# control-toolbox/CTDirect.jl

Measured on AMD Instinct MI355X. Metric: NLP callback evals/s (constraints+sparse Jac), N-step Goddard, 1/2/4/8 GPU, higher is better.
Workload: dtype f64; 1 GPU; cfg2_weak: goddard / gauss_legendre_2, 10000 time steps per GPU (global grid 10000 steps, time-step sharded); fused cons!+jac_coord! on HBM-resident x; BASELINE.json configs[1] per GPU; nvar_per_gpu=110004, ncon_per_gpu=90004, nnzj_per_gpu=1110028

## Files before the change

### ctdirect.jl_amd/csrc/ctd_engine.hip

```cpp
#include <hip/hip_runtime.h>
#include <hip/hiprtc.h>
#include <dlfcn.h>

#include <cstdio>
#include <functional>
#include <map>
#include <mutex>
#include <cstdlib>
#include <cstring>
#include <memory>
#include <new>
#include <string>
#include <vector>

#include "../../include/ctdirect_hip.h"
#include "ctd_host.hpp"
#include "ctd_kernels.hpp"
#include "ctd_hess_kernels.hpp"
#include "ctd_hess_step.hpp"
#include "ctd_iter_kernels.hpp"
#include "ctd_prod_kernels.hpp"
#include "ctd_hprod_kernels.hpp"
#include "ctd_kkt_kernels.hpp"
#include "ctd_diag_kernels.hpp"
// ... 322 lines not shown
template <class Enqueue>
static int32_t host_call(ctd_handle* h, std::initializer_list<Staged<const double>> in, Enqueue&& enqueue,
                         std::initializer_list<Staged<double>> out) {
    for (const auto& a : in) if (a.host) HIP_TRY(h, a.buf.ensure(a.n));
    for (const auto& a : out) if (a.host) HIP_TRY(h, a.buf.ensure(a.n));
    for (const auto& a : in) if (a.host) HIP_TRY(h, hipMemcpyAsync(a.buf.p, a.host, sizeof(double) * a.n, hipMemcpyHostToDevice, h->stream));
    if (const int32_t st = enqueue()) return st;
    for (const auto& a : out) if (a.host) HIP_TRY(h, hipMemcpyAsync(a.host, a.buf.p, sizeof(double) * a.n, hipMemcpyDeviceToHost, h->stream));
    HIP_TRY(h, hipStreamSynchronize(h->stream));
    return CTD_OK;
}

template <class K>
static int32_t enqueue_prod_units(ctd_handle* h, const char* fn, typename K::Params& a, int dirs, int jc, DevBuf<>& partial,
                                  const JitModule& jm, int f0, const double* x_dev, bool shard) {
    ProdParams& pp = K::prod(a);
    pp.nch = (int32_t)((dirs + jc - 1) / jc);
    const int64_t blocks = ((pp.unit_end - pp.unit_begin) * (int64_t)pp.nch + 255) / 256;
    if (blocks > 0x7fffffff) return fail(h, CTD_EINVAL, std::string(fn) + ": grid too large");
    pp.nblocks = (int32_t)blocks;
    const int32_t st = partial.grow(h, blocks * kMaxNV, fn);
    if (st) return st;
    pp.partial = partial.p;
    hipError_t e = hipErrorInvalidValue;
    if (h->rt) {
        void* args[] = {&a, &x_dev};
        e = jit_launch(jm.f[f0], (int)blocks, 256, 0, h->stream, args);
        if (e == hipSuccess) e = jit_launch(jm.f[f0 + 1], 1, 64, 0, h->stream, args);
    }
    for_problem(h->model.problem, [&](auto tag) {
        using P = typename decltype(tag)::type;
        if constexpr (K::kShardForm)
            e = shard ? launch_prod_units<P, K, true>(a, x_dev, h->stream) : launch_prod_units<P, K, false>(a, x_dev, h->stream);
        else e = launch_prod_units<P, K, false>(a, x_dev, h->stream);
    });
    if (e != hipSuccess) return fail(h, CTD_EHIP, std::string(fn) + ": kernel launch: " + hipGetErrorString(e));
    return CTD_OK;
}

extern "C" {

const char* ctd_strerror(int32_t st) {
    switch (st) {
        case CTD_OK: return "ok";
        case CTD_EINVAL: return "invalid argument";
        case CTD_EGRID: return "given time grid is not strictly increasing";
        case CTD_ESCHEME: return "unknown discretization method";
        case CTD_EPATTERN: return "sparsity pattern not available";
        case CTD_EPROBLEM: return "problem not in the compiled registry";
        case CTD_ENODEVICE: return "no HIP device bound to this handle (there is no CPU fallback)";
        case CTD_EHIP: return "HIP runtime error";
        case CTD_ENOMEM: return "out of memory";
        default: return "unknown status";
    }
}

const char* ctd_last_error(const ctd_handle* h) { return h ? h->err.c_str() : g_create_err.c_str(); }

int32_t ctd_create(const ctd_desc* desc, ctd_handle** out) {
    if (!desc || !out) return fail(nullptr, CTD_EINVAL, "ctd_create: null argument");
    *out = nullptr;
    struct Del { void operator()(ctd_handle* p) const { if (p) destroy_handle(p); } };
    std::unique_ptr<ctd_handle, Del> h(new (std::nothrow) ctd_handle());
    if (!h) return fail(nullptr, CTD_ENOMEM, "ctd_create: out of memory");
    HostDesc hd{desc->problem, desc->scheme, desc->pattern_mode, desc->grid_size, desc->time_grid, desc->time_grid_len,
                desc->control_steps > 1 ? desc->control_steps : 1, desc->value_order};
    if (desc->reserved0 != 0) return fail(nullptr, CTD_EINVAL, "ctd_create: ctd_desc.reserved0 must be 0 (zero-initialise the descriptor: memset / ctd_desc d = {0})");
    std::string err;
    int st;
    try {
        st = build_model(hd, h->model, err);
    } catch (const std::bad_alloc&) {
        return fail(nullptr, CTD_ENOMEM, "ctd_create: out of memory while building the model");
    }
    if (st) return fail(nullptr, st, err);
    const Model& mo = h->model;
    if (!runtime_ocp(mo.problem)) {
        const char* bad = nullptr;
        for_problem(mo.problem, [&](auto tag) {
            using P = typename decltype(tag)::type;
            for_scheme<true>(mo.L, [&](auto t) { bad = static_layout_mismatch<P, t.sc, t.s>(mo.L); });
        });
        if (bad) return fail(nullptr, CTD_EINVAL, std::string("ctd_create: the static layout of the kernel instantiation differs from the model's layout in field '") + bad + "'");
    }
    if (mo.L.cs > 3 && desc->device >= 0 && !runtime_ocp(mo.problem))
        return fail(nullptr, CTD_EINVAL, "ctd_create: control_steps > 3 needs an OCP registered at run time (ctd_register_ocp); the compiled registry holds the midpoint kernels for 1, 2 and 3 controls per step");
    h->step_begin = desc->step_begin;
    h->step_end = desc->step_end;
    if (h->step_begin == 0 && h->step_end == 0) h->step_end = mo.L.N;
    if (h->step_begin < 0 || h->step_end > mo.L.N || h->step_begin >= h->step_end)
        return fail(nullptr, CTD_EINVAL, "ctd_create: shard [step_begin, step_end) is not inside [0, N)");
    h->tile = env_int("CTD_TILE", 0);
    h->lean_ok = env_int("CTD_LEAN", 1) ? 1 : 0;
    if (h->tile <= 0) h->tile = default_tile(mo, h->step_end - h->step_begin);
    int maxb = 256;
    for_problem(mo.problem, [&](auto tag) { maxb = decltype(tag)::type::MAXB; });
    h->rt = runtime_ocp(mo.problem);
    if (h->rt) maxb = h->rt->maxb;
    h->block = env_int("CTD_BLOCK", 0);
    if (h->block <= 0) {
        h->block = 256;
        const int64_t ntl = (h->step_end - h->step_begin + h->tile - 1) / h->tile;
        if (ntl <= 512 && mo.nch_dyn <= 1 && mo.Lseg > 0 && 320 / mo.Lseg > 256 / mo.Lseg && mo.Lseg * (320 / mo.Lseg) * 10 >= 320 * 9) h->block = 320;
    }
    if (h->block < 64 || (h->block % 64)) h->block = 256;
    if (h->block > maxb) h->block = maxb;
    mo.fill_kparams(h->kp, h->step_begin, h->step_end, h->tile);
    h->lds_bytes = (size_t)lds_doubles(h->kp) * sizeof(double);
    const int debug_stop = env_int("CTD_DEBUG_STOP", 0);
    const size_t lds_cap = h->rt ? 64 * 1024 : 80 * 1024;
    while (h->lds_bytes > lds_cap && h->tile > 1) {
        h->tile = (h->tile + 1) / 2;
        mo.fill_kparams(h->kp, h->step_begin, h->step_end, h->tile);
        h->lds_bytes = (size_t)lds_doubles(h->kp) * sizeof(double);
    }
    const bool long_mid = mo.L.sc == SC_MIDPOINT && mo.L.cs == 1;
    if (desc->device >= 0 && !h->rt && env_int("CTD_TILE", 0) <= 0 && mo.nch_dyn <= 1 && (mo.L.sc == SC_IRK || long_mid) && h->tile >= 16) {
        DeviceGuard dgq(desc->device);
        if (dgq.err == hipSuccess) {
            auto resident = [&](int tile, size_t& lds) {
                KParams kq;
                mo.fill_kparams(kq, h->step_begin, h->step_end, tile);
                lds = (size_t)lds_doubles(kq) * sizeof(double);
                int r = 0;
                for_problem(mo.problem, [&](auto tag) { r = occupancy_cons_jac<typename decltype(tag)::type>(kq, h->block, lds); });
                (void)hipGetLastError();
                return r;
            };
            size_t l0 = 0;
            const int r0 = resident(h->tile, l0);
            const int64_t ns = h->step_end - h->step_begin, cap = 256 * (int64_t)r0;
            if (r0 > 0 && (ns + h->tile - 1) / h->tile >= env_int("CTD_LONG_GRID_ROUNDS", 8) * cap && maxb >= 512 && env_int("CTD_BLOCK", 0) <= 0 &&
                env_int("CTD_LONG_GRID", 1)) {
                int tbest = h->tile;
                for (int tt = h->tile + 1; tt <= 256; ++tt) {
                    KParams kq;
                    mo.fill_kparams(kq, h->step_begin, h->step_end, tt);
                    if ((size_t)lds_doubles(kq) * sizeof(double) > (long_mid ? 74u : 64u) * 1024) break;
                    tbest = tt;
                }
                if (tbest > h->tile) {
                    h->tile = tbest;
                    h->block = 512;
                    mo.fill_kparams(h->kp, h->step_begin, h->step_end, h->tile);
                    h->lds_bytes = (size_t)lds_doubles(h->kp) * sizeof(double);
                }
            } else if (mo.L.sc == SC_IRK && r0 > 0 && (ns + h->tile - 1) / h->tile > cap) {
                int tmax = 48;
                for (; tmax > h->tile; --tmax) { size_t l = 0; if (resident(tmax, l) >= r0 && l <= lds_cap) break; }
                const int64_t rounds = (ns + (int64_t)tmax * cap - 1) / ((int64_t)tmax * cap);
                const int64_t tb = (ns + rounds * cap - 1) / (rounds * cap);
                if (tb > h->tile && tb <= tmax) {
                    h->tile = (int)tb;
                    mo.fill_kparams(h->kp, h->step_begin, h->step_end, h->tile);
                    h->lds_bytes = (size_t)lds_doubles(h->kp) * sizeof(double);
                }
            }
        }
    }
    h->grid = h->kp.ntiles + h->kp.has_edge;
    h->kp.debug_stop = debug_stop;
    h->out_mb = 8.0 * ((double)(h->step_end - h->step_begin) * (mo.L.cb + mo.Lseg + (double)mo.L.nv * mo.vr)) / 1.0e6;
    h->kp.wt_store = h->out_mb <= kWtMB ? 1 : 0;
    h->device = desc->device;
    if (h->device >= 0) {
        int ndev = 0;
        if (hipGetDeviceCount(&ndev) != hipSuccess || h->device >= ndev)
            return fail(nullptr, CTD_ENODEVICE, "ctd_create: HIP device not available");
        ctd_handle* hp = h.get();
        if (h->lds_bytes > 160 * 1024) return fail(nullptr, CTD_EINVAL, "ctd_create: tile does not fit the 160 KiB LDS");
        DeviceGuard dg_(hp->device); HIP_TRY(nullptr, dg_.err);
        if (desc->stream_mode == CTD_STREAM_GIVEN) { hp->stream = (hipStream_t)desc->stream; hp->own_stream = false; }
        else { HIP_TRY(nullptr, hipStreamCreateWithFlags(&hp->stream, hipStreamNonBlocking)); hp->own_stream = true; }
        HIP_TRY(nullptr, upload(hp->d_tau, mo.tau));
        HIP_TRY(nullptr, upload(hp->d_tmpl, mo.tmpl));
        HIP_TRY(nullptr, upload(hp->d_vtmpl, mo.vtmpl));
        HIP_TRY(nullptr, upload(hp->d_edge_idx, mo.edge_idx));
        HIP_TRY(nullptr, upload(hp->d_edge_code, mo.edge_code));
        hp->kp.tau = hp->d_tau.p;
        hp->kp.tmpl = hp->d_tmpl.p;
        hp->kp.vtmpl = hp->d_vtmpl.p;
        {
            const int S = mo.L.s, r_dyn = S * mo.nch_dyn, r_path = mo.nch_path;
            int lgT = 0;
            while ((1 << lgT) < hp->tile) ++lgT;
            const int leadbase = (((r_dyn + r_path) << lgT) + 63) & ~63;
            const int early_lanes = mo.n_early + mo.c_early + mo.L.nv * mo.vr_early;
            if (env_int("CTD_EARLY", 0) && mo.n_early > 0 && !hp->rt && mo.fused && hp->tile <= 32 && leadbase + 64 <= hp->block && early_lanes <= 64 &&
                mo.n_late > 0 && mo.n_late <= hp->block) {
                HIP_TRY(nullptr, upload(hp->d_pos, mo.pos_order));
                hp->kp.pos = hp->d_pos.p;
                hp->kp.n_late = mo.n_late; hp->kp.n_early = mo.n_early; hp->kp.c_early = mo.c_early; hp->kp.vr_early = mo.vr_early;
                hp->kp.div_late = make_fastdiv((uint32_t)mo.n_late);
            }
        }
        hp->kp.edge_idx = hp->d_edge_idx.p;
        hp->kp.edge_code = hp->d_edge_code.p;
        hp->obj_blocks = 256;
        HIP_TRY(nullptr, hp->d_partial.ensure(hp->obj_blocks));
        HIP_TRY(nullptr, hp->d_obj.ensure(1));
        HIP_TRY(nullptr, hipEventCreate(&hp->ev0));
        HIP_TRY(nullptr, hipEventCreate(&hp->ev1));
        if (hp->rt) {
            if (hp->lds_bytes > 64 * 1024) return fail(nullptr, CTD_EINVAL, "ctd_create: one step of this run-time OCP does not fit 64 KiB of LDS");
            const int32_t jst = jit_load(hp, JIT_FIRST);
            if (jst) return jst;
        }
        {
            const bool direct = mo.fused && mo.L.sc != SC_TRAPEZE;
            const int mt = env_int("CTD_MULTI_TILE", 0);
            if (!direct && mt > 0 && kMultiTileLoop && !hp->rt) {
                int per_cu = mt > 1 ? mt : 0, cus = 256;
                if (hipDeviceGetAttribute(&cus, hipDeviceAttributeMultiprocessorCount, hp->device) != hipSuccess) cus = 256;
                if (per_cu == 0) {
                    if (hp->rt) {
                        if (hipModuleOccupancyMaxActiveBlocksPerMultiprocessor(&per_cu, hp->jit[JIT_FIRST].f[0], hp->block, hp->lds_bytes) != hipSuccess) per_cu = 0;
                    } else {
                        for_problem(mo.problem, [&](auto tag) {
                            using P = typename decltype(tag)::type;
                            per_cu = occupancy_cons_jac<P>(hp->kp, hp->block, hp->lds_bytes);
                        });
                    }
                }
                const int64_t cap = (int64_t)per_cu * cus - hp->kp.has_edge;
                if (cap > 0 && hp->kp.ntiles > cap) {
                    hp->kp.wg_stride = (int)cap;
                    hp->grid = hp->kp.wg_stride + hp->kp.has_edge;
                }
            }
        }
    }
    *out = h.release();
    return CTD_OK;
}

int32_t ctd_register_ocp(const ctd_ocp_def* def, int32_t* problem_id) {
    if (!def || !problem_id) return fail(nullptr, CTD_EINVAL, "ctd_register_ocp: null argument");
    std::string err;
    int id = -1;
    const int st = register_runtime_ocp(def, &id, err);
    if (st) return fail(nullptr, st, "ctd_register_ocp: " + err);
    *problem_id = id;
    return CTD_OK;
}

int32_t ctd_ocp_source(int32_t problem_id, char* buf, int64_t cap) {
// ... 1587 lines not shown
```

### ctdirect.jl_amd/csrc/ctd_kernel_body.hpp

```cpp
#pragma once
#include "ctd_layout.hpp"


namespace ctd {

#if defined(CTD_SUBSTAMPS) && defined(__HIP_DEVICE_COMPILE__)
#ifndef CTD_SUB_WAVE0
#define CTD_SUB_WAVE0 0
#endif
#define CTD_SUB(kp, id)                                                                                              \
    do {                                                                                                             \
        __builtin_amdgcn_sched_barrier(0);                                                                           \
        __builtin_amdgcn_s_waitcnt(0);                                                                               \
        if ((kp).stamps && (threadIdx.x & 63) == 0 && threadIdx.x >= 64 * CTD_SUB_WAVE0 && threadIdx.x < 64 * CTD_SUB_WAVE0 + 128) \
            (kp).stamps[(size_t)gridDim.x * 12 + ((size_t)blockIdx.x * 2 + (threadIdx.x >> 6) - CTD_SUB_WAVE0) * 8 + (id)] = clock64(); \
        __builtin_amdgcn_sched_barrier(0);                                                                           \
    } while (0)
#else
#define CTD_SUB(kp, id) do { } while (0)
#endif
#if defined(CTD_SUBSTAMPS_EMIT) && defined(__HIP_DEVICE_COMPILE__)
#define CTD_SUBE(kp, id)                                                                                             \
    do {                                                                                                             \
        __builtin_amdgcn_sched_barrier(0);                                                                           \
// ... 1521 lines not shown
#pragma unroll
                        for (int u = 0; u < 4; ++u) {
                            const int s = s0 + u * par;
                            if (s < nreg) emit_store(&out[s * Ls + k], a[u] * b[u] + beta, kp.wt_store);
                        }
                    }
                }
            } else {
                uint32_t code = (hp && tid < Ls) ? pre_->b : (tid < Ls ? cx.codes[tid] : 0u);
                int q = 0;
                for (int k = tid; k < Ls; k += nthr, ++q) {
                    uint32_t nxt = 0u;
                    bool have = false;
                    if constexpr (NB > 1) {
                        if (hp && q < NB - 1) {
                            have = true;
#pragma unroll
                            for (int e = 0; e < NB - 1; ++e)
                                if (e == q) nxt = pre_->more[e];
                        }
                    }
                    if (!have) nxt = k + nthr < Ls ? cx.codes[k + nthr] : 0u;
                    const int bt = code_beta(code);
                    const double beta = bt == 0 ? 0.0 : (bt == 1 ? 1.0 : -1.0);
                    const double* pc = cx.rec + (sl0 - code_crec(code)) * stride + R.oC + code_ci(code);
                    const double* pd = cx.rec + (sl0 - code_drec(code)) * stride + code_di(code);
                    const int last = nreg - 1;
                    for (int s0 = 0; s0 < nreg; s0 += 4) {
                        double a[4], b[4];
#pragma unroll
                        for (int u = 0; u < 4; ++u) {
                            const int s = s0 + u < last ? s0 + u : last;
                            a[u] = pc[s * stride];
                            b[u] = pd[s * stride];
                        }
#pragma unroll
                        for (int u = 0; u < 4; ++u)
                            if (s0 + u < nreg) emit_store(&out[(s0 + u) * Ls + k], a[u] * b[u] + beta, kp.wt_store);
                    }
                    code = nxt;
                }
            }
        }
    }
    CTD_SUBE(kp, 2);
    if (kp.vr > 0) {
        const int vr = kp.vr;
        const int par = (int)fast_div((uint32_t)nthr, kp.div_vr);
#pragma unroll
        for (int kk = 0; kk < P::NV; ++kk) {
            double* out = out_vals<B>(kp, bl) + kp.vcol_base[kk] + cx.a * (int64_t)vr;
            const uint32_t* codes = cx.vcodes + kk * vr;
            if (par >= 1) {
                if (tid < par * vr) {
                    const int g = (int)fast_div((uint32_t)tid, kp.div_vr), k = tid - g * vr;
                    const uint32_t code = hp ? pre_->v[kk] : codes[k];
                    const double* pc = cx.rec + (slot0 + g) * stride + R.oC + code_ci(code);
                    const double* pd = cx.rec + (slot0 + g) * stride + code_di(code);
                    const int adv = par * stride;
                    if (LEAN || k >= kp.vr_early)
                        for (int s = g; s < nsteps; s += par, pc += adv, pd += adv) emit_store(&out[s * vr + k], (*pc) * (*pd), kp.wt_store);
                }
            } else {
                for (int k = tid; k < vr; k += nthr) {
                    const uint32_t code = codes[k];
                    const double* pc = cx.rec + slot0 * stride + R.oC + code_ci(code);
                    const double* pd = cx.rec + slot0 * stride + code_di(code);
                    for (int s = 0; s < nsteps; ++s, pc += stride, pd += stride) emit_store(&out[s * vr + k], (*pc) * (*pd), kp.wt_store);
                }
            }
        }
    }
    CTD_SUBE(kp, 3);
}
template <class P, int SC, int S, int NB = 1, bool B = false, bool LEAN = false>
CTD_HD void phase_emit(const KParams& kp, const BlockCtx& cx, int tid, int nthr, const EmitPreT<NB>* pre = nullptr,
                       const BatchLd bl = BatchLd{}) {
    if (pre != nullptr) phase_emit_impl<P, SC, S, NB, B, LEAN>(kp, cx, tid, nthr, *pre, pre->have != 0, bl);
    else phase_emit_impl<P, SC, S, NB, B, LEAN>(kp, cx, tid, nthr, EmitPreT<NB>{}, false, bl);
}

}

#if !defined(__HIPCC_RTC__)
#include "ctd_problems.hpp"
#include "ctd_sym_registry.hpp"
#endif
```

### ctdirect.jl_amd/csrc/ctd_kernels.hpp

```cpp
#pragma once
#if !defined(__HIPCC_RTC__)
#include <hip/hip_runtime.h>
#include <hip/hip_ext.h>
#endif

#include "ctd_kernel_body.hpp"
#if !defined(__HIPCC_RTC__)
#include "ctd_problems.hpp"
#endif

namespace ctd {

#ifndef CTD_MULTI_TILE_LOOP
#define CTD_MULTI_TILE_LOOP 0
#endif
constexpr bool kMultiTileLoop = CTD_MULTI_TILE_LOOP != 0;

template <bool DBG>
__device__ __forceinline__ void ctd_stamp(const KParams& kp, int slot) {
    if constexpr (DBG) {
        if (kp.stamps && threadIdx.x == 0) {
            unsigned long long* p = kp.stamps + ((size_t)blockIdx.x * 6 + slot) * 2;
            p[0] = wall_clock64();
            p[1] = clock64();
// ... 41 lines not shown

template <class P, int SC, int S, bool DBG, bool B = false, bool LEAN = false>
__device__ __forceinline__ void cons_jac_body(const KParams& kp, const double* __restrict__ xu, int block, double* ctd_lds,
                                              const BatchLd bl = BatchLd{}) {
    if constexpr (B) xu += batch_member() * bl.ldx;
    ctd_pin_kernargs<SC == SC_IRK ? S : 0, LEAN>(kp, xu);
    ctd_stamp<DBG>(kp, 0);
    if (DBG && kp.debug_stop == 1) return;
    const int tid = (int)threadIdx.x, nthr = (int)blockDim.x;
    if constexpr (DirectTile<P, SC>::value) {
        const BlockCtx cx = make_direct_ctx<LEAN>(kp, block, ctd_lds, xu, LV<P, SC, S, LEAN>::blk(kp), LEAN ? P::NV : -1);
        const EmitPre pre = emit_prefetch<P, 1, LEAN>(kp, cx, tid, nthr);
        ctd_stamp<DBG>(kp, 1);
        phase_eval<P, SC, S, RegEval<P, SC, S>::value, 1, B, LEAN>(kp, cx, tid, nthr, &pre, bl);
        ctd_pin_emit_kernargs<LEAN>(kp);
        __syncthreads();
        ctd_stamp<DBG>(kp, 2);
        ctd_stamp<DBG>(kp, 3);
        if (DBG && kp.debug_stop >= 2 && kp.debug_stop <= 4) return;
        phase_emit<P, SC, S, 1, B, LEAN>(kp, cx, tid, nthr, &pre, bl);
        ctd_stamp<DBG>(kp, 4);
        if (DBG && kp.stamps) {
            __builtin_amdgcn_s_waitcnt(0);
            __syncthreads();
            ctd_stamp<DBG>(kp, 5);
        }
        return;
    }
    BlockCtx cx = make_ctx<LEAN>(kp, block, ctd_lds);
    constexpr int NB = EmitN<P, SC, S>::value;
    EmitPreT<NB> pre = {};
    const bool use_pre = !cx.is_edge && !codes_staged(kp);
    if (use_pre) pre = emit_prefetch<P, NB, LEAN>(kp, cx, tid, nthr);
    phase_load<P, SC, S, true, LEAN>(kp, cx, xu, tid, nthr);
    const int nblk = kp.ntiles + kp.has_edge;
    for (;;) {
        __syncthreads();
        ctd_stamp<DBG>(kp, 1);
        if (DBG && kp.debug_stop == 2) return;
        phase_eval<P, SC, S, false, 1, B, LEAN>(kp, cx, tid, nthr, nullptr, bl);
        ctd_pin_emit_kernargs<LEAN>(kp);
        __syncthreads();
        ctd_stamp<DBG>(kp, 2);
        if (DBG && kp.debug_stop == 3) return;
        if (!Dirs<P>::FUSED && !fin_folded<P, SC, S>(cx)) {
            phase_fin<P, SC, S>(kp, cx, tid, nthr);
            __syncthreads();
        }
        if (SC == SC_TRAPEZE) {
            phase_fin2<P, SC, S>(kp, cx, tid, nthr);
            __syncthreads();
        }
        ctd_stamp<DBG>(kp, 3);
        if (DBG && kp.debug_stop == 4) return;
        block += kp.wg_stride;
        const bool more = kMultiTileLoop && kp.wg_stride > 0 && !cx.is_edge && block < nblk;
        BlockCtx nx = cx;
        TileIn tin{0.0, 0.0, 0.0};
        if (more) {
            nx = make_ctx<LEAN>(kp, block, ctd_lds);
            tin = load_issue<P>(kp, nx, xu, tid, nthr);
        }
        phase_emit_impl<P, SC, S, NB, B, LEAN>(kp, cx, tid, nthr, pre, use_pre, bl);
        ctd_stamp<DBG>(kp, 4);
        if (!more) break;
        load_commit<P, SC, S>(kp, nx, xu, tin, tid, nthr);
        cx = nx;
    }
    if (DBG && kp.stamps) {
        __builtin_amdgcn_s_waitcnt(0);
        __syncthreads();
        ctd_stamp<DBG>(kp, 5);
    }
}

template <class P, int SC, int S> struct MinWaves {
    static constexpr int value = (P::NX <= 12 && !(SC == SC_MIDPOINT && S > 1)) ? 4 : 1;
};

template <class P, int SC, int S, bool DBG, bool LEAN = false>
__global__ void __launch_bounds__(P::MAXB, (MinWaves<P, SC, S>::value)) cons_jac_kernel(const KParams kp, const double* __restrict__ xu) {
    extern __shared__ double ctd_lds[];
    cons_jac_body<P, SC, S, DBG, false, LEAN>(kp, xu, (int)blockIdx.x, ctd_lds);
}
template <class P, int SC, int S>
__global__ void __launch_bounds__(P::MAXB, (MinWaves<P, SC, S>::value)) cons_jac_batch_kernel(const KParams kp, const double* __restrict__ xu,
                                                                                          const BatchLd bl) {
    extern __shared__ double ctd_lds[];
    cons_jac_body<P, SC, S, false, true>(kp, xu, (int)blockIdx.x, ctd_lds, bl);
}

struct ObjParams {
    Layout L;
    const double* tau;
    int64_t unit_begin, unit_end;
    int32_t add_mayer;
    double* partial;
    double* out;
    int32_t nblocks;
    const XHalo* halo;
    XNear near;
    int64_t ldx;
};

template <class P> __device__ double obj_time(const ObjParams& op, const double* v, int64_t i) {
    const double t0 = (P::IT0 >= 0) ? v[P::IT0 >= 0 ? P::IT0 : 0] : op.L.t0;
    const double tf = (P::ITF >= 0) ? v[P::ITF >= 0 ? P::ITF : 0] : op.L.tf;
    const double tau = op.tau ? op.tau[i] : (double)i / (double)op.L.N;
    return t0 + tau * (tf - t0);
}

template <class P, int SC>
__device__ double lagrange_unit(const ObjParams& op, const double* __restrict__ xu, const double* v, int64_t i) {
    constexpr int n = P::NX, m = P::NU;
    const Layout& L = op.L;
    const double* base = xu + i * (int64_t)L.blk;
    const int64_t gn = (i + 1) * (int64_t)L.blk;
    const double* nxt = ((op.halo && i + 1 >= op.unit_end) ? xnear(op.near, xu, gn) : xu) + gn;
    double x[n > 0 ? n : 1], u[m > 0 ? m : 1];
    if (SC == SC_TRAPEZE) {
        double w;
        if (i == 0) w = (obj_time<P>(op, v, 1) - obj_time<P>(op, v, 0)) / 2.0;
        else if (i == L.N) w = (obj_time<P>(op, v, L.N) - obj_time<P>(op, v, L.N - 1)) / 2.0;
        else w = (obj_time<P>(op, v, i + 1) - obj_time<P>(op, v, i - 1)) / 2.0;
        for (int c = 0; c < n; ++c) x[c] = base[c];
        for (int c = 0; c < m; ++c) u[c] = base[n + c];
        return w * P::template lagrange<double>(obj_time<P>(op, v, i), x, u, v);
    }
    const double ti = obj_time<P>(op, v, i), tip1 = obj_time<P>(op, v, i + 1);
    const double h = tip1 - ti;
    if (SC == SC_MIDPOINT) {
        if (L.cs > 1) {
            const double hi = h / (double)L.cs;
            for (int c = 0; c < n; ++c) x[c] = 0.5 * (base[c] + nxt[c]);
            double val = 0.0;
            for (int j = 1; j <= L.cs; ++j) {
                for (int c = 0; c < m; ++c) u[c] = base[n + (j - 1) * m + c];
                const double term = hi * P::template lagrange<double>(ti + ((double)j - 0.5) * hi, x, u, v);
                val = (j == 1) ? term : val + term;
            }
            return val;
        }
        for (int c = 0; c < m; ++c) u[c] = base[n + c];
        if (L.euler == 0) {
            for (int c = 0; c < n; ++c) x[c] = 0.5 * (base[c] + nxt[c]);
            return h * P::template lagrange<double>(0.5 * (ti + tip1), x, u, v);
        }
        for (int c = 0; c < n; ++c) x[c] = (L.euler == 1) ? base[c] : nxt[c];
        return h * P::template lagrange<double>(L.euler == 1 ? ti : tip1, x, u, v);
    }
    const double* K = base + n + L.cu;
    double local = 0.0;
    for (int j = 0; j < L.s; ++j) {
        for (int c = 0; c < n; ++c) {
            double xc = base[c];
            for (int l = 0; l < L.s; ++l) xc = xc + h * L.a[3 * j + l] * K[l * n + c];
            x[c] = xc;
        }
        const double* U = base + n + (L.stagewise ? j * m : 0);
        for (int c = 0; c < m; ++c) u[c] = U[c];
        const double term = L.b[j] * P::template lagrange<double>(ti + L.c[j] * h, x, u, v);
        local = (j == 0) ? term : local + term;
    }
    return h * local;
}

// ... 315 lines not shown
    const int lane = threadIdx.x & 63, wave = threadIdx.x >> 6;
    for (int k = 0; k < nv; ++k) {
        double a = gv[k];
        for (int off = 32; off > 0; off >>= 1) a += __shfl_down(a, off, 64);
        if (lane == 0) wsum[wave][k] = a;
    }
    __syncthreads();
    if (threadIdx.x == 0)
        for (int k = 0; k < nv; ++k) {
            double sacc = 0.0;
            for (int w = 0; w < (int)(blockDim.x >> 6); ++w) sacc += wsum[w][k];
            gp.partial[((size_t)mb * gp.nblocks + block) * kMaxNV + k] = sacc;
        }
}
template <class P, int SC, int S>
__global__ void __launch_bounds__(256) __attribute__((amdgpu_waves_per_eu(2))) grad_units_kernel(const GradParams gp, const double* __restrict__ xu) {
    __shared__ double wsum[4][kMaxNV];
    const int64_t mb = batch_member();
    grad_units_body<P, SC, S>(gp, xu + mb * gp.ldx, (int)blockIdx.x, wsum, mb);
}

template <class P>
__device__ __forceinline__ void grad_finish_body(const GradParams& gp, const double* __restrict__ xu, int64_t mb = 0) {
    if (threadIdx.x >= 64) return;
    constexpr int n = P::NX, nv = P::NV;
    const Layout& L = gp.L;
    const double* part = gp.partial + (size_t)mb * gp.nblocks * kMaxNV;
    double* const g = gp.g + mb * gp.ldg;
    double gvs[nv > 0 ? nv : 1];
    for (int k = 0; k < nv; ++k) {
        double sacc = 0.0;
        for (int b = threadIdx.x; b < gp.nblocks; b += 64) sacc += part[(size_t)b * kMaxNV + k];
        for (int off = 32; off > 0; off >>= 1) sacc += __shfl_down(sacc, off, 64);
        gvs[k] = sacc;
    }
    if (threadIdx.x != 0) return;
    if (P::HAS_MAYER && (gp.owns_first || gp.owns_last)) {
        double x0[n > 0 ? n : 1], xf[n > 0 ? n : 1], v[nv > 0 ? nv : 1], g0x[n > 0 ? n : 1], gfx[n > 0 ? n : 1], gmv[nv > 0 ? nv : 1];
        const double* b0 = grad_block(gp, xu, 0);
        const double* bf = grad_block(gp, xu, L.N);
        for (int c = 0; c < n; ++c) { x0[c] = b0[c]; xf[c] = bf[c]; g0x[c] = 0.0; gfx[c] = 0.0; }
        for (int k = 0; k < nv; ++k) { v[k] = xu[L.v_off + k]; gmv[k] = 0.0; }
        mayer_partials<P, 0>(x0, xf, v, g0x, gfx, gmv);
        for (int c = 0; c < n; ++c) {
            if (gp.owns_first) g[c] += g0x[c];
            if (gp.owns_last) g[L.N * (int64_t)L.blk + c] += gfx[c];
        }
        if (gp.owns_last) for (int k = 0; k < nv; ++k) gvs[k] += gmv[k];
    }
    for (int k = 0; k < nv; ++k) g[L.v_off + k] = gvs[k];
}
template <class P>
__global__ void grad_finish_kernel(const GradParams gp, const double* __restrict__ xu) {
    if (blockIdx.x != 0) return;
    const int64_t mb = batch_member();
    grad_finish_body<P>(gp, xu + mb * gp.ldx, mb);
}

#if !defined(__HIPCC_RTC__)
template <class P>
hipError_t launch_grad(const GradParams& gp, const double* xu, int grid, hipStream_t st, int batch) {
    const dim3 g(grid > 0 ? grid : 1, batch);
    if (grid > 0)
        for_scheme<false>(gp.L, [&](auto t) { grad_units_kernel<P, t.sc, t.s><<<g, 256, 0, st>>>(gp, xu); });
    grad_finish_kernel<P><<<dim3(1, batch), 64, 0, st>>>(gp, xu);
    return hipGetLastError();
}

#endif

#if !defined(__HIPCC_RTC__)
template <class P, int SC, int S, bool DBG, bool LEAN>
hipError_t launch_variant_dbg(const KParams& kp, const double* xu, int grid, int block, size_t lds_bytes, hipStream_t st,
                              hipEvent_t e0, hipEvent_t e1) {
    if (lds_bytes > 64 * 1024) {
        hipError_t e = hipFuncSetAttribute((const void*)cons_jac_kernel<P, SC, S, DBG, LEAN>, hipFuncAttributeMaxDynamicSharedMemorySize,
                                           (int)lds_bytes);
        if (e != hipSuccess) return e;
    }
    if (e0 || e1) hipExtLaunchKernelGGL((cons_jac_kernel<P, SC, S, DBG, LEAN>), dim3(grid), dim3(block), lds_bytes, st, e0, e1, 0, kp, xu);
    else cons_jac_kernel<P, SC, S, DBG, LEAN><<<grid, block, lds_bytes, st>>>(kp, xu);
    return hipGetLastError();
}
template <class P, int SC, int S>
hipError_t launch_variant(const KParams& kp, const double* xu, int grid, int block, size_t lds_bytes, hipStream_t st,
                          hipEvent_t e0, hipEvent_t e1, int lean_ok) {
    const bool dbg = kp.stamps || kp.debug_stop;
    constexpr bool kHasLean = DirectTile<P, SC>::value || SC == SC_IRK;
    if constexpr (kHasLean) {
        if (lean_ok && kp.halo == nullptr && kp.n_early == 0) {
            if (dbg) return launch_variant_dbg<P, SC, S, true, true>(kp, xu, grid, block, lds_bytes, st, e0, e1);
            return launch_variant_dbg<P, SC, S, false, true>(kp, xu, grid, block, lds_bytes, st, e0, e1);
        }
    }
    if (dbg) return launch_variant_dbg<P, SC, S, true, false>(kp, xu, grid, block, lds_bytes, st, e0, e1);
    return launch_variant_dbg<P, SC, S, false, false>(kp, xu, grid, block, lds_bytes, st, e0, e1);
}

template <class P>
hipError_t launch_cons_jac(const KParams& kp, const double* xu, int grid, int block, size_t lds_bytes, hipStream_t st,
                           hipEvent_t e0, hipEvent_t e1, int lean_ok) {
    hipError_t e = hipErrorInvalidValue;
    for_scheme<true>(kp.L, [&](auto t) { e = launch_variant<P, t.sc, t.s>(kp, xu, grid, block, lds_bytes, st, e0, e1, lean_ok); });
    return e;
}

template <class P, int SC, int S>
int occupancy_variant(int block, size_t lds_bytes) {
    int nb = 0;
    if (lds_bytes > 64 * 1024 &&
        hipFuncSetAttribute((const void*)cons_jac_kernel<P, SC, S, false>, hipFuncAttributeMaxDynamicSharedMemorySize, (int)lds_bytes) != hipSuccess)
        return 0;
    if (hipOccupancyMaxActiveBlocksPerMultiprocessor(&nb, cons_jac_kernel<P, SC, S, false>, block, lds_bytes) != hipSuccess) return 0;
    return nb;
}
template <class P, int SC, int S>
hipError_t launch_variant_batch(const KParams& kp, const double* xu, const BatchLd& bl, int grid, int block, size_t lds_bytes, hipStream_t st,
                                int batch) {
    if (lds_bytes > 64 * 1024) {
        hipError_t e = hipFuncSetAttribute((const void*)cons_jac_batch_kernel<P, SC, S>, hipFuncAttributeMaxDynamicSharedMemorySize, (int)lds_bytes);
        if (e != hipSuccess) return e;
    }
    cons_jac_batch_kernel<P, SC, S><<<dim3(grid, batch), block, lds_bytes, st>>>(kp, xu, bl);
    return hipGetLastError();
}
template <class P>
hipError_t launch_cons_jac_batch(const KParams& kp, const double* xu, const BatchLd& bl, int grid, int block, size_t lds_bytes,
                                 hipStream_t st, int batch) {
    hipError_t e = hipErrorInvalidValue;
    for_scheme<true>(kp.L, [&](auto t) { e = launch_variant_batch<P, t.sc, t.s>(kp, xu, bl, grid, block, lds_bytes, st, batch); });
    return e;
}

template <class P>
int occupancy_cons_jac(const KParams& kp, int block, size_t lds_bytes) {
    int nb = 0;
    for_scheme<true>(kp.L, [&](auto t) { nb = occupancy_variant<P, t.sc, t.s>(block, lds_bytes); });
    return nb;
}

template <class P>
hipError_t launch_obj(const ObjParams& op, const double* xu, int grid, int block, hipStream_t st, int batch) {
    const dim3 g(grid > 0 ? grid : 1, batch);
    if (grid > 0)
        for_scheme<false>(op.L, [&](auto t) { obj_partial_kernel<P, t.sc><<<g, block, 0, st>>>(op, xu); });
    obj_finish_kernel<P><<<dim3(1, batch), 64, 0, st>>>(op, xu);
    return hipGetLastError();
}

#define CTD_INSTANTIATE_LAUNCHERS(P)                                                                                       \
    template hipError_t launch_cons_jac<P>(const KParams&, const double*, int, int, size_t, hipStream_t, hipEvent_t, \
                                           hipEvent_t, int);                                                                 \
    template hipError_t launch_cons_jac_batch<P>(const KParams&, const double*, const BatchLd&, int, int, size_t, hipStream_t, int); \
    template hipError_t launch_obj<P>(const ObjParams&, const double*, int, int, hipStream_t, int);                  \
    template int occupancy_cons_jac<P>(const KParams&, int, size_t);                                                 \
    template hipError_t launch_grad<P>(const GradParams&, const double*, int, hipStream_t, int);
#define CTD_EXTERN_LAUNCHERS(P)                                                                                            \
    extern template hipError_t launch_cons_jac<P>(const KParams&, const double*, int, int, size_t, hipStream_t,      \
                                                  hipEvent_t, hipEvent_t, int);                                              \
    extern template hipError_t launch_cons_jac_batch<P>(const KParams&, const double*, const BatchLd&, int, int, size_t, hipStream_t, \
                                                        int);                                                                      \
    extern template hipError_t launch_obj<P>(const ObjParams&, const double*, int, int, hipStream_t, int);          \
    extern template int occupancy_cons_jac<P>(const KParams&, int, size_t);                                         \
    extern template hipError_t launch_grad<P>(const GradParams&, const double*, int, hipStream_t, int);

#endif

}
```

### profiles/resource_usage.py

```python
import argparse
import os
import re
import subprocess
from concurrent.futures import ThreadPoolExecutor

ROOT = os.path.dirname(os.path.dirname(os.path.abspath(__file__)))
CSRC = os.path.join(ROOT, "ctdirect.jl_amd", "csrc")
HIPCC = os.environ.get("HIPCC", "/opt/rocm/bin/hipcc")
KERNELS = ("jprod_kernel", "jtprod_units_kernel", "jtprod_finish_kernel", "hprod_units_kernel", "hprod_finish_kernel")
PRODUCTS = [(p, p) for p in ("quadrotor", "quadrotor12", "goddard_all", "double_integrator_free_t0_tf", "goddard",
                             "double_integrator_path", "estimate_initial_condition", "estimate_rotation_rate",
                             "least_squares_constraint", "stagewise_scalar")]
HPROD = [("double_integrator_free_t0_tf", "double_integrator_freet0tf"), ("double_integrator_path", "double_integrator_path"),
         ("estimate_initial_condition", "estimate_initial_condition"), ("estimate_rotation_rate", "estimate_rotation_rate"),
         ("goddard", "goddard"), ("goddard_all", "goddard_all"), ("least_squares_constraint", "least_squares_with_constraint"),
         ("quadrotor", "quadrotor"), ("quadrotor12", "quadrotor12"), ("stagewise_scalar", "stagewise_scalar")]
DIAG_KERNELS = ("hdiag_units_kernel", "hdiag_finish_kernel", "jsq_cols_units_kernel", "jsq_cols_finish_kernel", "jsq_rows_kernel")
SCHEMES = ("trapeze", "midpoint / Euler", "Gauss-Legendre 1", "Gauss-Legendre 2", "Gauss-Legendre 3")
FIELDS = (("vgpr", r" VGPRs: (\d+)"), ("agpr", r"AGPRs: (\d+)"), ("scratch", r"ScratchSize \[bytes/lane\]: (\d+)"),
          ("waves", r"Occupancy \[waves/SIMD\]: (\d+)"))


def remarks(stem, prefix="ctd_pkern_", kernels=KERNELS):
    r = subprocess.run([HIPCC, "--offload-arch=gfx950", "-O3", "-std=c++17", "-ffp-contract=off", "--cuda-device-only",
                        "-Rpass-analysis=kernel-resource-usage", "-c", f"{prefix}{stem}.hip", "-o", os.devnull],
                       cwd=CSRC, capture_output=True, text=True)
    if r.returncode:
        raise SystemExit(r.stderr[-4000:])
    out, cur = [], None
    for line in r.stderr.splitlines():
        m = re.search(r"Function Name: (\S+)", line)
        if m:
            k = re.search("|".join(kernels), m.group(1))
            cur = {"kernel": k.group(0), "shard": bool(re.search(r"Lb1EE+v", m.group(1)))} if k else None
            continue
        if cur is None:
            continue
        for key, pat in FIELDS:
            m = re.search(pat, line)
            if m:
                cur[key] = int(m.group(1))
        if "LDS Size" in line:
            out.append(cur)
            cur = None
    return out


def write(log, problems, table, hprod):
    path = os.path.join(ROOT, "profiles", log)
    with open(path) as f:
        head = [l for l in f if l.startswith("#")]
    lines = []
    for stem, name in problems:
        ks = [k for k in table[stem] if k["kernel"].startswith("hprod") == hprod]
        for k in sorted(ks, key=lambda k: k["shard"]):
            assert k["scratch"] == 0, (name, k)
            ag = f" agpr={k['agpr']}" if hprod else ""
            lines.append(f"{name} {k['kernel']}{' shard' if k['shard'] else ''} vgpr={k['vgpr']}{ag} scratch=0 waves={k['waves']}\n")
    with open(path, "w") as f:
        f.writelines(head + lines)
    print(path, len(lines), "kernels")


def write_diag(table):
    path = os.path.join(ROOT, "profiles", "diag_resources.md")
    with open(path) as f:
        text = f.read()
    head = text[:text.index("| problem |")] if "| problem |" in text else text
    cell = lambda k: f"{k['vgpr']} + {k['agpr']} | {k['scratch']} | {k['waves']}"
    lines = ["| problem | scheme | hdiag VGPR + AGPR | scratch B/lane | waves/SIMD | jsq_cols VGPR + AGPR | scratch B/lane | waves/SIMD "
             "| jsq_rows VGPR + AGPR | scratch B/lane | waves/SIMD |\n", "|---|---|---|---|---|---|---|---|---|---|---|\n"]
    for stem, name in HPROD:
        by = {kn: [k for k in table[stem] if k["kernel"] == kn] for kn in DIAG_KERNELS}
        for k in table[stem]:
            assert k["scratch"] == 0, (name, k)
        assert all(len(by[kn]) == 5 for kn in ("hdiag_units_kernel", "jsq_cols_units_kernel", "jsq_rows_kernel")), name
        for i, sch in enumerate(SCHEMES):
            lines.append(f"| {name} | {sch} | {cell(by['hdiag_units_kernel'][i])} | {cell(by['jsq_cols_units_kernel'][i])} | "
                         f"{cell(by['jsq_rows_kernel'][i])} |\n")
        lines.append(f"| {name} | finish | {cell(by['hdiag_finish_kernel'][0])} | {cell(by['jsq_cols_finish_kernel'][0])} | | | |\n")
    with open(path, "w") as f:
        f.write(head)
        f.writelines(lines)
    print(path, len(lines) - 2, "rows")


def main():
    ap = argparse.ArgumentParser()
    ap.add_argument("--jobs", type=int, default=8)
    args = ap.parse_args()
    stems = [s for s, _ in PRODUCTS]
    with ThreadPoolExecutor(args.jobs) as ex:
        table = dict(zip(stems, ex.map(remarks, stems)))
    write("products_resource_usage.log", PRODUCTS, table, False)
    write("hprod_resource_usage.log", HPROD, table, True)
    with ThreadPoolExecutor(args.jobs) as ex:
        dtable = dict(zip(stems, ex.map(lambda s: remarks(s, "ctd_dkern_", DIAG_KERNELS), stems)))
    write_diag(dtable)


if __name__ == "__main__":
    main()
```

Before: 177,400 evals/s.

## Add compile-time-specialised static emit kernel for fused cons/jac on unsharded IRK grids

Adds a cons_jac_static_kernel whose emit phase uses compile-time segment lengths, vr, and thread count. This replaces the runtime-indexed template emit with chunked register-prefetched loads and stores, and fixes the write-through choice as a template parameter. It is meant to remove runtime index arithmetic, branches and scalar loads behind the barrier, and to batch global stores. The kernel is enabled by default only for compiled OCPs with a full, unsharded step range, and adds a host check that the static geometry matches the model. It costs more instantiations and code size, and adds an env override for write-through stores.

```diff
diff --git a/ctdirect.jl_amd/csrc/ctd_emit_static.hpp b/ctdirect.jl_amd/csrc/ctd_emit_static.hpp
--- /dev/null
+++ b/ctdirect.jl_amd/csrc/ctd_emit_static.hpp
@@ -0,0 +1,164 @@
+#pragma once
+
+namespace ctd {
+
+template <class P, int SC, int S> struct StaticEmit {
+    using SL = StaticLayout<P, SC, S>;
+    static constexpr int n = SL::n, m = SL::m, nv = SL::nv, p = SL::p, s = SL::s, cb = SL::cb;
+    static constexpr bool stagewise = SC == SC_IRK && S >= 2;
+    static constexpr int cu = SL::cu(stagewise);
+    static constexpr int Lseg = SC == SC_IRK ? n * (2 * n + s * n + p) + cu * (s * n + p) + s * n * (n + s * n) : 0;
+    static constexpr int vr = nv > 0 ? cb : 0;
+    static constexpr bool offered = DirectTile<P, SC>::value && SC == SC_IRK && Lseg > 0;
+    template <int NTHR> static constexpr bool fits() { return offered && Lseg <= NTHR && cb <= NTHR; }
+    static constexpr bool wants320 = Lseg > 0 && 320 / (Lseg > 0 ? Lseg : 1) > 256 / (Lseg > 0 ? Lseg : 1) &&
+                                     Lseg * (320 / (Lseg > 0 ? Lseg : 1)) * 10 >= 320 * 9;
+    template <int NTHR> static constexpr bool built() { return fits<NTHR>() && P::MAXB >= NTHR && (NTHR == 256 || (NTHR == 320 && wants320)); }
+};
+template <class P, int SC, int S> inline const char* static_emit_mismatch(const Layout& L, int Lseg, int vr) {
+    using SE = StaticEmit<P, SC, S>;
+    if (SC != SC_IRK) return nullptr;
+    if (Lseg <= 0) return nullptr;
+    if (SC == SC_IRK && S >= 2 && !L.stagewise) return nullptr;
+    if (Lseg != SE::Lseg) return "Lseg";
+    if (vr != SE::vr) return "vr";
+    return nullptr;
+}
+
+template <class P, int SC, int S, int NTHR>
+CTD_HD EmitPre emit_prefetch_static(const KParams& kp, int tid) {
+    using SE = StaticEmit<P, SC, S>;
+    EmitPre pre;
+    pre.b = 0u; pre.eidx = 0; pre.have = 1; pre.kpos = 0; pre.eb = 0u; pre.ek = 0; pre.more[0] = 0u;
+    pre.b = kp.tmpl[(uint32_t)tid % (uint32_t)SE::Lseg];
+#pragma unroll
+    for (int kk = 0; kk < kMaxNV; ++kk) {
+        pre.v[kk] = 0u;
+        if constexpr (SE::vr > 0) { if (kk < P::NV) pre.v[kk] = kp.vtmpl[kk * SE::vr + (int)((uint32_t)tid % (uint32_t)SE::vr)]; }
+    }
+    return pre;
+}
+
+template <int CH, int PAR, int STRIDE>
+CTD_HD void se_load(const double* p, int c0, int jmax, double* v) {
+#pragma unroll
+    for (int u = 0; u < CH; ++u) {
+        int j = (c0 + u) * PAR;
+        j = j < jmax ? j : jmax;
+        v[u] = p[j * STRIDE];
+    }
+}
+template <int K, int CH, int PITCH, bool WT>
+CTD_HD void se_store_case(double* out, const double* v, int kf, bool tail) {
+    if (kf == K) {
+#pragma unroll
+        for (int u = 0; u < K; ++u) emit_store(out + (int64_t)u * PITCH, v[u], WT);
+        if (tail) emit_store(out + (int64_t)K * PITCH, v[K], WT);
+        return;
+    }
+    if constexpr (K > 0) se_store_case<K - 1, CH, PITCH, WT>(out, v, kf, tail);
+}
+template <int CH, int PITCH, bool WT>
+CTD_HD void se_store(double* out, const double* v, int kf, bool tail) {
+    if (kf >= CH) {
+#pragma unroll
+        for (int u = 0; u < CH; ++u) emit_store(out + (int64_t)u * PITCH, v[u], WT);
+        return;
+    }
+    se_store_case<CH - 1, CH, PITCH, WT>(out, v, kf, tail);
+}
+
+template <class P, int SC, int S, int NTHR, bool WT>
+CTD_HD void phase_emit_static(const KParams& kp, const BlockCtx& cx, int tid, const EmitPre& pre) {
+    using SE = StaticEmit<P, SC, S>;
+    static_assert(SE::template fits<NTHR>(), "a period of this instantiation exceeds the workgroup");
+    constexpr RecLayout R = RL<P, SC, S>::R;
+    constexpr int stride = R.stride;
+    constexpr int cb = SE::cb, Ls = SE::Lseg, vr = SE::vr, NV = P::NV;
+    constexpr int parA = NTHR / cb, parB = NTHR / Ls, parC = vr > 0 ? NTHR / vr : 1;
+    constexpr int CHA = 2, CHB = 8, CHC = 2;
+    static_assert(2 * CHB + CHA + 2 * kMaxNV * CHC <= 48, "the first chunk of every stream is held in registers at once");
+    const int nsteps = (int)(cx.b - cx.a), slot0 = (int)(cx.a - cx.lo);
+    const int64_t ra = cx.a > kp.reg_first ? cx.a : kp.reg_first, rb = cx.b < kp.reg_last ? cx.b : kp.reg_last;
+    const int nreg = (int)(rb - ra), sl0 = (int)(ra - cx.lo);
+    const bool doA = kp.c != nullptr && nsteps > 0, doB = kp.vals != nullptr && nreg > 0, doC = kp.vals != nullptr && vr > 0 && nsteps > 0;
+    const int gA = (int)((uint32_t)tid / (uint32_t)cb), rA = tid - gA * cb;
+    const int gB = (int)((uint32_t)tid / (uint32_t)Ls);
+    const int gC = vr > 0 ? (int)((uint32_t)tid / (uint32_t)(vr > 0 ? vr : 1)) : 0;
+    const bool actA = tid < parA * cb, actB = tid < parB * Ls, actC = vr > 0 && tid < parC * vr;
+    const int nfA = nsteps / parA, remA = nsteps - nfA * parA;
+    const int nfB = nreg > 0 ? nreg / parB : 0, remB = nreg > 0 ? nreg - nfB * parB : 0;
+    const int nfC = nsteps / parC, remC = nsteps - nfC * parC;
+    const double* srcA = cx.rec + (slot0 + gA) * stride + R.oR + rA;
+    const uint32_t code = pre.b;
+    const int bt = code_beta(code);
+    const double beta = bt == 0 ? 0.0 : (bt == 1 ? 1.0 : -1.0);
+    const double* pcB = cx.rec + (sl0 + gB - code_crec(code)) * stride + R.oC + code_ci(code);
+    const double* pdB = cx.rec + (sl0 + gB - code_drec(code)) * stride + code_di(code);
+    const double* pcC[NV > 0 ? NV : 1];
+    const double* pdC[NV > 0 ? NV : 1];
+#pragma unroll
+    for (int kk = 0; kk < NV; ++kk) {
+        pcC[kk] = cx.rec + (slot0 + gC) * stride + R.oC + code_ci(pre.v[kk]);
+        pdC[kk] = cx.rec + (slot0 + gC) * stride + code_di(pre.v[kk]);
+    }
+    double* outA = doA ? kp.c + cx.a * (int64_t)cb + tid : nullptr;
+    double* outB = doB ? kp.vals + kp.seg_base + (ra - kp.reg_first) * (int64_t)Ls + tid : nullptr;
+    double* outC[NV > 0 ? NV : 1];
+#pragma unroll
+    for (int kk = 0; kk < NV; ++kk) outC[kk] = doC ? kp.vals + kp.vcol_base[kk] + cx.a * (int64_t)vr + tid : nullptr;
+
+    double vA[CHA], aB[CHB], bB[CHB], aC[NV > 0 ? NV : 1][CHC], bC[NV > 0 ? NV : 1][CHC];
+    if (doA) se_load<CHA, parA, stride>(srcA, 0, nsteps - 1 - gA, vA);
+    if (doB) {
+        se_load<CHB, parB, stride>(pcB, 0, nreg - 1 - gB, aB);
+        se_load<CHB, parB, stride>(pdB, 0, nreg - 1 - gB, bB);
+    }
+    if (doC) {
+#pragma unroll
+        for (int kk = 0; kk < NV; ++kk) {
+            se_load<CHC, parC, stride>(pcC[kk], 0, nsteps - 1 - gC, aC[kk]);
+            se_load<CHC, parC, stride>(pdC[kk], 0, nsteps - 1 - gC, bC[kk]);
+        }
+    }
+    if (doA && actA) se_store<CHA, parA * cb, WT>(outA, vA, nfA, gA < remA);
+    if (doB) {
+#pragma unroll
+        for (int u = 0; u < CHB; ++u) aB[u] = aB[u] * bB[u] + beta;
+        if (actB) se_store<CHB, parB * Ls, WT>(outB, aB, nfB, gB < remB);
+    }
+    if (doC) {
+#pragma unroll
+        for (int kk = 0; kk < NV; ++kk) {
+#pragma unroll
+            for (int u = 0; u < CHC; ++u) aC[kk][u] = aC[kk][u] * bC[kk][u];
+            if (actC) se_store<CHC, parC * (vr > 0 ? vr : 1), WT>(outC[kk], aC[kk], nfC, gC < remC);
+        }
+    }
+    if (doA)
+        for (int c0 = CHA; c0 * parA < nsteps; c0 += CHA) {
+            se_load<CHA, parA, stride>(srcA, c0, nsteps - 1 - gA, vA);
+            if (actA) se_store<CHA, parA * cb, WT>(outA + (int64_t)c0 * (parA * cb), vA, nfA - c0, gA < remA);
+        }
+    if (doB)
+        for (int c0 = CHB; c0 * parB < nreg; c0 += CHB) {
+            se_load<CHB, parB, stride>(pcB, c0, nreg - 1 - gB, aB);
+            se_load<CHB, parB, stride>(pdB, c0, nreg - 1 - gB, bB);
+#pragma unroll
+            for (int u = 0; u < CHB; ++u) aB[u] = aB[u] * bB[u] + beta;
+            if (actB) se_store<CHB, parB * Ls, WT>(outB + (int64_t)c0 * (parB * Ls), aB, nfB - c0, gB < remB);
+        }
+    if (doC) {
+#pragma unroll
+        for (int kk = 0; kk < NV; ++kk)
+            for (int c0 = CHC; c0 * parC < nsteps; c0 += CHC) {
+                se_load<CHC, parC, stride>(pcC[kk], c0, nsteps - 1 - gC, aC[kk]);
+                se_load<CHC, parC, stride>(pdC[kk], c0, nsteps - 1 - gC, bC[kk]);
+#pragma unroll
+                for (int u = 0; u < CHC; ++u) aC[kk][u] = aC[kk][u] * bC[kk][u];
+                if (actC) se_store<CHC, parC * (vr > 0 ? vr : 1), WT>(outC[kk] + (int64_t)c0 * (parC * (vr > 0 ? vr : 1)), aC[kk], nfC - c0, gC < remC);
+            }
+    }
+}
+
+}
diff --git a/ctdirect.jl_amd/csrc/ctd_engine.hip b/ctdirect.jl_amd/csrc/ctd_engine.hip
--- a/ctdirect.jl_amd/csrc/ctd_engine.hip
+++ b/ctdirect.jl_amd/csrc/ctd_engine.hip
@@ -428,6 +428,13 @@
             for_scheme<true>(mo.L, [&](auto t) { bad = static_layout_mismatch<P, t.sc, t.s>(mo.L); });
         });
         if (bad) return fail(nullptr, CTD_EINVAL, std::string("ctd_create: the static layout of the kernel instantiation differs from the model's layout in field '") + bad + "'");
+        if (mo.pattern_mode == 0 && mo.order == 0) {
+            for_problem(mo.problem, [&](auto tag) {
+                using P = typename decltype(tag)::type;
+                for_scheme<true>(mo.L, [&](auto t) { bad = static_emit_mismatch<P, t.sc, t.s>(mo.L, mo.Lseg, mo.vr); });
+            });
+            if (bad) return fail(nullptr, CTD_EINVAL, std::string("ctd_create: the static emit geometry of the kernel instantiation differs from the model's in '") + bad + "'");
+        }
     }
     if (mo.L.cs > 3 && desc->device >= 0 && !runtime_ocp(mo.problem))
         return fail(nullptr, CTD_EINVAL, "ctd_create: control_steps > 3 needs an OCP registered at run time (ctd_register_ocp); the compiled registry holds the midpoint kernels for 1, 2 and 3 controls per step");
@@ -438,6 +445,9 @@
         return fail(nullptr, CTD_EINVAL, "ctd_create: shard [step_begin, step_end) is not inside [0, N)");
     h->tile = env_int("CTD_TILE", 0);
     h->lean_ok = env_int("CTD_LEAN", 1) ? 1 : 0;
+    if (h->lean_ok && env_int("CTD_STATIC_EMIT", 1) && !runtime_ocp(mo.problem) && mo.pattern_mode == 0 && mo.order == 0 &&
+        h->step_begin == 0 && h->step_end == mo.L.N)
+        h->lean_ok |= 2;
     if (h->tile <= 0) h->tile = default_tile(mo, h->step_end - h->step_begin);
     int maxb = 256;
     for_problem(mo.problem, [&](auto tag) { maxb = decltype(tag)::type::MAXB; });
@@ -508,6 +518,7 @@
     h->kp.debug_stop = debug_stop;
     h->out_mb = 8.0 * ((double)(h->step_end - h->step_begin) * (mo.L.cb + mo.Lseg + (double)mo.L.nv * mo.vr)) / 1.0e6;
     h->kp.wt_store = h->out_mb <= kWtMB ? 1 : 0;
+    if (const int wt = env_int("CTD_WT_STORE", -1); wt >= 0) h->kp.wt_store = wt ? 1 : 0;
     h->device = desc->device;
     if (h->device >= 0) {
         int ndev = 0;
diff --git a/ctdirect.jl_amd/csrc/ctd_kernel_body.hpp b/ctdirect.jl_amd/csrc/ctd_kernel_body.hpp
--- a/ctdirect.jl_amd/csrc/ctd_kernel_body.hpp
+++ b/ctdirect.jl_amd/csrc/ctd_kernel_body.hpp
@@ -1627,6 +1627,8 @@
 
 }
 
+#include "ctd_emit_static.hpp"
+
 #if !defined(__HIPCC_RTC__)
 #include "ctd_problems.hpp"
 #include "ctd_sym_registry.hpp"
diff --git a/ctdirect.jl_amd/csrc/ctd_kernels.hpp b/ctdirect.jl_amd/csrc/ctd_kernels.hpp
--- a/ctdirect.jl_amd/csrc/ctd_kernels.hpp
+++ b/ctdirect.jl_amd/csrc/ctd_kernels.hpp
@@ -147,6 +147,46 @@
 __global__ void __launch_bounds__(P::MAXB, (MinWaves<P, SC, S>::value)) cons_jac_kernel(const KParams kp, const double* __restrict__ xu) {
     extern __shared__ double ctd_lds[];
     cons_jac_body<P, SC, S, DBG, false, LEAN>(kp, xu, (int)blockIdx.x, ctd_lds);
+}
+template <class P, int SC, int S, bool DBG, int NTHR, bool WT>
+__device__ __forceinline__ void cons_jac_static_body(const KParams& kp, const double* __restrict__ xu, int block, double* ctd_lds) {
+    if (__builtin_expect(block < kp.has_edge, 0)) {
+        cons_jac_body<P, SC, S, DBG, false, true>(kp, xu, block, ctd_lds);
+        return;
+    }
+#if defined(__HIP_DEVICE_COMPILE__)
+    asm volatile("" ::"s"(kp.has_edge), "s"(kp.T), "s"(kp.HL), "s"(kp.HH), "s"(kp.step_begin), "s"(kp.step_end), "s"(kp.L.N),
+                 "s"(kp.L.v_off), "s"(kp.L.stagewise), "s"(kp.L.euler), "s"(kp.tau), "s"(kp.L.t0), "s"(kp.L.tf), "s"(xu),
+                 "s"(kp.tmpl), "s"(kp.vtmpl));
+#endif
+    ctd_stamp<DBG>(kp, 0);
+    if (DBG && kp.debug_stop == 1) return;
+    const int tid = (int)threadIdx.x;
+    BlockCtx cx = make_direct_ctx<true>(kp, block, ctd_lds, xu, LV<P, SC, S, true>::blk(kp), P::NV);
+    cx.is_edge = 0;
+    cx.edge_part = 0;
+    const EmitPre pre = emit_prefetch_static<P, SC, S, NTHR>(kp, tid);
+    ctd_stamp<DBG>(kp, 1);
+    phase_eval<P, SC, S, RegEval<P, SC, S>::value, 1, false, true>(kp, cx, tid, NTHR, &pre, BatchLd{});
+#if defined(__HIP_DEVICE_COMPILE__)
+    asm volatile("" ::"s"(kp.c), "s"(kp.vals), "s"(kp.seg_base), "s"(kp.reg_first), "s"(kp.reg_last), "s"(kp.vcol_base[0]));
+#endif
+    __syncthreads();
+    ctd_stamp<DBG>(kp, 2);
+    ctd_stamp<DBG>(kp, 3);
+    if (DBG && kp.debug_stop >= 2 && kp.debug_stop <= 4) return;
+    phase_emit_static<P, SC, S, NTHR, WT>(kp, cx, tid, pre);
+    ctd_stamp<DBG>(kp, 4);
+    if (DBG && kp.stamps) {
+        __builtin_amdgcn_s_waitcnt(0);
+        __syncthreads();
+        ctd_stamp<DBG>(kp, 5);
+    }
+}
+template <class P, int SC, int S, bool DBG, int NTHR, bool WT>
+__global__ void __launch_bounds__(NTHR, (MinWaves<P, SC, S>::value)) cons_jac_static_kernel(const KParams kp, const double* __restrict__ xu) {
+    extern __shared__ double ctd_lds[];
+    cons_jac_static_body<P, SC, S, DBG, NTHR, WT>(kp, xu, (int)blockIdx.x, ctd_lds);
 }
 template <class P, int SC, int S>
 __global__ void __launch_bounds__(P::MAXB, (MinWaves<P, SC, S>::value)) cons_jac_batch_kernel(const KParams kp, const double* __restrict__ xu,
@@ -628,10 +668,39 @@
     else cons_jac_kernel<P, SC, S, DBG, LEAN><<<grid, block, lds_bytes, st>>>(kp, xu);
     return hipGetLastError();
 }
+template <class P, int SC, int S, int NTHR>
+hipError_t launch_static(const KParams& kp, const double* xu, int grid, size_t lds_bytes, hipStream_t st, hipEvent_t e0, hipEvent_t e1,
+                         bool dbg, bool& done) {
+    done = false;
+    if constexpr (StaticEmit<P, SC, S>::template built<NTHR>()) {
+        using SE = StaticEmit<P, SC, S>;
+        if (kp.Lseg != SE::Lseg || kp.vr != SE::vr || (SC == SC_IRK && S >= 2 && !kp.L.stagewise)) return hipSuccess;
+        done = true;
+        auto go = [&](auto kern) -> hipError_t {
+            if (lds_bytes > 64 * 1024) {
+                hipError_t e = hipFuncSetAttribute((const void*)kern, hipFuncAttributeMaxDynamicSharedMemorySize, (int)lds_bytes);
+                if (e != hipSuccess) return e;
+            }
+            if (e0 || e1) hipExtLaunchKernelGGL(kern, dim3(grid), dim3(NTHR), lds_bytes, st, e0, e1, 0, kp, xu);
+            else kern<<<grid, NTHR, lds_bytes, st>>>(kp, xu);
+            return hipGetLastError();
+        };
+        if (dbg) return kp.wt_store ? go(cons_jac_static_kernel<P, SC, S, true, NTHR, true>) : go(cons_jac_static_kernel<P, SC, S, true, NTHR, false>);
+        return kp.wt_store ? go(cons_jac_static_kernel<P, SC, S, false, NTHR, true>) : go(cons_jac_static_kernel<P, SC, S, false, NTHR, false>);
+    }
+    return hipSuccess;
+}
 template <class P, int SC, int S>
 hipError_t launch_variant(const KParams& kp, const double* xu, int grid, int block, size_t lds_bytes, hipStream_t st,
                           hipEvent_t e0, hipEvent_t e1, int lean_ok) {
     const bool dbg = kp.stamps || kp.debug_stop;
+    if ((lean_ok & 3) == 3 && kp.halo == nullptr && kp.n_early == 0 && (block == 256 || block == 320)) {
+        bool done = false;
+        const hipError_t e = block == 256 ? launch_static<P, SC, S, 256>(kp, xu, grid, lds_bytes, st, e0, e1, dbg, done)
+                                          : launch_static<P, SC, S, 320>(kp, xu, grid, lds_bytes, st, e0, e1, dbg, done);
+        if (done) return e;
+    }
+    lean_ok &= 1;
     constexpr bool kHasLean = DirectTile<P, SC>::value || SC == SC_IRK;
     if constexpr (kHasLean) {
         if (lean_ok && kp.halo == nullptr && kp.n_early == 0) {
diff --git a/profiles/resource_usage.py b/profiles/resource_usage.py
--- a/profiles/resource_usage.py
+++ b/profiles/resource_usage.py
@@ -85,10 +85,92 @@
     print(path, len(lines) - 2, "rows")
 
 
+CONS_JAC = (("cfg2", "goddard", "GoddardOCP", 2, 2, 320), ("cfg3", "double_integrator_path", "DoubleIntegratorPathOCP", 1, 1, 256),
+            ("cfg4", "goddard", "GoddardOCP", 2, 3, 256))
+
+
+def cons_jac_counts(stem):
+    r = subprocess.run([HIPCC, "--offload-arch=gfx950", "-O3", "-std=c++17", "-ffp-contract=off", "--cuda-device-only", "-S",
+                        "-Rpass-analysis=kernel-resource-usage", f"ctd_kern_{stem}.hip", "-o", "-"], cwd=CSRC, capture_output=True, text=True)
+    if r.returncode:
+        raise SystemExit(r.stderr[-4000:])
+    res, cur = {}, None
+    pats = (("sgpr", r"TotalSGPRs: (\d+)"), ("vgpr", r" VGPRs: (\d+)"), ("scratch", r"ScratchSize \[bytes/lane\]: (\d+)"),
+            ("waves", r"Occupancy \[waves/SIMD\]: (\d+)"), ("sgpr_spill", r"SGPRs Spill: (\d+)"), ("vgpr_spill", r"VGPRs Spill: (\d+)"))
+    for line in r.stderr.splitlines():
+        m = re.search(r"Function Name: (\S+)", line)
+        if m:
+            cur = res.setdefault(m.group(1), {})
+            continue
+        if cur is not None:
+            for key, pat in pats:
+                m = re.search(pat, line)
+                if m:
+                    cur[key] = int(m.group(1))
+    name, body = None, []
+    for line in r.stdout.splitlines():
+        m = re.match(r"^(_ZN3ctd\w*cons_jac\w*):", line)
+        if m:
+            name, body = m.group(1), []
+            continue
+        if name is None:
+            continue
+        m = re.search(r"; codeLenInByte = (\d+)", line)
+        if m and name in res:
+            ins = [l.split()[0] for l in body if l.startswith("\t") and (l.lstrip().startswith(";;#ASMSTART") or not l.lstrip().startswith((".", ";")))]
+            b0 = next((i for i, x in enumerate(ins) if x == "s_barrier"), None)
+            sec = []
+            if b0 is not None:
+                e0 = next((i for i in range(b0, len(ins)) if ins[i] in ("s_endpgm", ";;#ASMSTART")), len(ins))
+                sec = ins[b0 + 1:e0]
+                if e0 < len(ins) and ins[e0] == ";;#ASMSTART":
+                    hi = max((i for i, x in enumerate(sec) if x.startswith("s_load")), default=-1)
+                    lo, i, gap = hi, hi - 1, 0
+                    while i >= 0 and gap <= 3:
+                        if sec[i].startswith("s_load"):
+                            lo, gap = i, 0
+                        else:
+                            gap += 1
+                        i -= 1
+                    if hi >= 0 and len(sec) - hi <= 4:
+                        sec = sec[:lo]
+            ins = [x for x in ins if x != ";;#ASMSTART"]
+            res[name].update(code_bytes=int(m.group(1)), instructions=len(ins), sec_instructions=len(sec),
+                             sec_branches=sum(x.startswith(("s_branch", "s_cbranch")) for x in sec),
+                             sec_scalar_loads=sum(x.startswith("s_load") for x in sec),
+                             sec_stores=sum(x.startswith("global_store") for x in sec))
+            name = None
+            continue
+        body.append(line)
+    return res
+
+
+def cons_jac_table():
+    print("| workload | kernel | code bytes | instructions | behind the barrier: instructions | branches | scalar loads | stores "
+          "| SGPRs | VGPRs | SGPR / VGPR spills | scratch | waves/SIMD |")
+    print("|---|---|---|---|---|---|---|---|---|---|---|---|---|")
+    cache = {}
+    for cfg, stem, ocp, sc, s, lanes in CONS_JAC:
+        res = cache.setdefault(stem, cons_jac_counts(stem))
+        tag = f"{len(ocp)}{ocp}ELi{sc}ELi{s}E"
+        for label, suffix in (("lean", f"cons_jac_kernelINS_{tag}Lb0ELb1EEE"), (f"static, {lanes} lanes, write-through", f"cons_jac_static_kernelINS_{tag}Lb0ELi{lanes}ELb1EEE")):
+            k = [v for n, v in res.items() if suffix in n]
+            if not k:
+                print(f"| {cfg} | {label} | not built |")
+                continue
+            k = k[0]
+            assert k["scratch"] == 0, (cfg, label, k)
+            print(f"| {cfg} | {label} | {k['code_bytes']} | {k['instructions']} | {k['sec_instructions']} | {k['sec_branches']} | {k['sec_scalar_loads']} "
+                  f"| {k['sec_stores']} | {k['sgpr']} | {k['vgpr']} | {k['sgpr_spill']} / {k['vgpr_spill']} | {k['scratch']} | {k['waves']} |")
+
+
 def main():
     ap = argparse.ArgumentParser()
     ap.add_argument("--jobs", type=int, default=8)
+    ap.add_argument("--cons-jac", action="store_true", help="print the table of profiles/static_emit.md (lean and static-emit kernels of cfg2 / cfg3 / cfg4) and stop")
     args = ap.parse_args()
+    if args.cons_jac:
+        return cons_jac_table()
     stems = [s for s, _ in PRODUCTS]
     with ThreadPoolExecutor(args.jobs) as ex:
         table = dict(zip(stems, ex.map(remarks, stems)))
```

New measurement: 187,900 evals/s, median of 6. 1.06x the previous value.
